# KUIS-AI-Tekalp-Research-Group/video-compression

Hardware: AMD Instinct MI355X
Metric: frames/sec + bpp/PSNR on UVG 1080p GOP-8, 1/2/4/8 MI355X (higher is better)
Workload: dtype f32; 1 GPU; LHBDC 1080p GOP-8 inference, single lambda: 7 B-frames per GOP via Model.forward, 4 independent GOP(s) per GPU per step, hierarchy levels batched across them; gop=8, resolution=1920x1080, precision=fp32, parallelism=gop-shard x1, launch=hip-graph per GOP pass

## Files before the change

video-compression_amd/csrc/conv_split.h:

```cpp
#pragma once
#include "conv_dma.h"

typedef short bf16x8 __attribute__((ext_vector_type(8)));

template <int K> struct SplitUnits {
    static constexpr int TPU = 4;
    static constexpr int Q = (K / 2) * (K / 2);
    static constexpr int V = (K + 3) / 4;
    static constexpr int H = (K - 1 + 3) / 4;
    static constexpr int U = Q + V + H;
    static constexpr int type(int u) { return u < Q ? 0 : (u < Q + V ? 1 : 2); }
    static constexpr int ky0(int u) { return u < Q ? 2 * (u / (K / 2)) : (u < Q + V ? 4 * (u - Q) : K - 1); }
    static constexpr int kx0(int u) { return u < Q ? 2 * (u % (K / 2)) : (u < Q + V ? K - 1 : 4 * (u - Q - V)); }
    static constexpr int nvalid(int u)
    {
        return u < Q ? 4 : (u < Q + V ? (K - 4 * (u - Q) < 4 ? K - 4 * (u - Q) : 4) : (K - 1 - 4 * (u - Q - V) < 4 ? K - 1 - 4 * (u - Q - V) : 4));
    }
    static constexpr int ky(int u, int q)
    {
        const int qq = q < nvalid(u) ? q : nvalid(u) - 1;
        return type(u) == 0 ? ky0(u) + (qq >> 1) : (type(u) == 1 ? ky0(u) + qq : ky0(u));
    }
    static constexpr int kx(int u, int q)
    {
        const int qq = q < nvalid(u) ? q : nvalid(u) - 1;
        return type(u) == 0 ? kx0(u) + (qq & 1) : (type(u) == 1 ? kx0(u) : kx0(u) + qq);
    }
    static constexpr bool valid(int u, int q) { return q < nvalid(u); }
    static constexpr int cls(int u) { return type(u) * 4 + nvalid(u) - 1; }
    static constexpr int NCLS = 12;
    static constexpr int dy(int c, int q)
    {
        const int t = c / 4, nv = c % 4 + 1, qq = q < nv ? q : nv - 1;
        return t == 0 ? (qq >> 1) : (t == 1 ? qq : 0);
    }
    static constexpr int dx(int c, int q)
    {
        const int t = c / 4, nv = c % 4 + 1, qq = q < nv ? q : nv - 1;
        return t == 0 ? (qq & 1) : (t == 1 ? 0 : qq);
    }
    static constexpr bool covers_all()
    {
        int seen[K * K] = {};
        for (int u = 0; u < U; ++u)
            for (int q = 0; q < 4; ++q)
                if (valid(u, q)) ++seen[ky(u, q) * K + kx(u, q)];
        for (int i = 0; i < K * K; ++i)
            if (seen[i] != 1) return false;
        return true;
    }
    static_assert(covers_all(), "every tap in exactly one unit");
};

template <int K> struct SplitPairs {
    static constexpr int TPU = 2;
    static constexpr int HP = (K - 1) / 2;
    static constexpr int Q = HP * K;
    static constexpr int V = (K + 1) / 2;
    static constexpr int U = Q + V;
    static constexpr int type(int u) { return u < Q ? 2 : 1; }
    static constexpr int ky0(int u) { return u < Q ? u / HP : 2 * (u - Q); }
    static constexpr int kx0(int u) { return u < Q ? 2 * (u % HP) : K - 1; }
    static constexpr int nvalid(int u) { return u < Q ? 2 : (K - 2 * (u - Q) < 2 ? 1 : 2); }
    static constexpr int ky(int u, int q) { return type(u) == 1 ? ky0(u) + (q < nvalid(u) ? q : nvalid(u) - 1) : ky0(u); }
    static constexpr int kx(int u, int q) { return type(u) == 2 ? kx0(u) + (q < nvalid(u) ? q : nvalid(u) - 1) : kx0(u); }
    static constexpr bool valid(int u, int q) { return q < nvalid(u); }
    static constexpr int cls(int u) { return type(u) * 4 + nvalid(u) - 1; }
    static constexpr int NCLS = 12;
    static constexpr int dy(int c, int q)
    {
        const int t = c / 4, nv = c % 4 + 1, qq = q < nv ? q : nv - 1;
        return t == 1 ? qq : 0;
    }
    static constexpr int dx(int c, int q)
    {
        const int t = c / 4, nv = c % 4 + 1, qq = q < nv ? q : nv - 1;
        return t == 2 ? qq : 0;
    }
    static constexpr bool covers_all()
    {
        int seen[K * K] = {};
        for (int u = 0; u < U; ++u)
            for (int q = 0; q < 2; ++q)
                if (valid(u, q)) ++seen[ky(u, q) * K + kx(u, q)];
        for (int i = 0; i < K * K; ++i)
            if (seen[i] != 1) return false;
        return true;
    }
    static_assert(covers_all(), "every tap in exactly one unit");
};

template <int K, int CPL> struct SplitUnitsOf { typedef SplitUnits<K> type; };
template <int K> struct SplitUnitsOf<K, 2> { typedef SplitPairs<K> type; };

template <int K_, int NTW_, int CPL_ = 1, int TH_ = 16, int RING_ = 4, int KO_ = 0> struct SplitCfg {
    typedef typename SplitUnitsOf<K_, CPL_>::type UN;
    static_assert(UN::TPU * CPL_ == 4, "four k-groups of 8 channels per MFMA");
    static constexpr int K = K_, NTW = NTW_, CPL = CPL_, RING = RING_, KO = KO_, U = UN::U, PAD = K_ / 2;
    static constexpr int TH = TH_, TW = 32, BN = 16 * NTW_;
    static constexpr int WAVES = 8, WM = TH_ * 2 / 8, WN = NTW_;
    static_assert(WM * 8 == TH_ * 2, "the tile's 2 TH M-tiles split evenly over 8 waves");
    static constexpr int ROWS_IN = TH + K_ - 1, COLS = TW + K_ - 1, PIX = ROWS_IN * COLS;
    static constexpr int PXB = 48;
    static constexpr int PLANE_SLOTS = CPL_ == 1 ? 3 * PIX : (3 * PIX + 15) / 16 * 16;
    static constexpr int PLANE_B = PLANE_SLOTS * 16;
    static constexpr int NA = (CPL_ * PLANE_SLOTS + 511) / 512;
    static constexpr int A_BYTES = NA * 8192;
    static constexpr int FRAGS = 3 * NTW_;
    static constexpr int ROUNDS = (FRAGS + 7) / 8, LASTW = FRAGS - 8 * (ROUNDS - 1);
    static constexpr bool EXACT = LASTW == 4;
    static constexpr int SLOTB = EXACT ? FRAGS * 1024 : ROUNDS * 8192;
    static constexpr int nb(int grp) { return ROUNDS - ((EXACT && grp == 1) ? 1 : 0); }
    static constexpr int B_OFF = 2 * A_BYTES, BIAS_OFF = B_OFF + RING_ * SLOTB;
    static constexpr int LDS_FIXED = BIAS_OFF;
    static constexpr int D = RING_ - 2;
    static constexpr int WIN = U - D - 1, PPP = (NA + WIN - 1) / WIN;
    static_assert(WIN >= 1, "no issue window for the chunk image");
    static constexpr int piece_phase(int k) { return 1 + k / PPP; }
    static constexpr int nA(int u)
    {
        int n = 0;
        for (int k = 0; k < NA; ++k) n += piece_phase(k) == u;
        return n;
    }
    static constexpr int nwait(int u, int grp)
    {
        int n = 0;
        for (int j = u + 2 - D; j <= u; ++j) n += nA(((j % U) + U) % U) + nb(grp);
        return n;
    }
    static_assert(D >= 1 && nwait(U - 1, 0) <= 63, "vmcnt is a 6-bit counter");
};

template <class C, int NG, int T0 = 0, int T1 = C::WM>
__device__ __forceinline__ void split_epilogue_records(const ConvArgs &p, f32x4 (&acc)[C::WM][C::WN], const DmaTile &cur, int wave, int px, int q,
                                                       unsigned char *sc)
{
    constexpr int WM = C::WM, WN = C::WN, UNITS = 96 * NG, NJ = (UNITS + 63) / 64, NGRP = (T1 - T0) * (WN / NG);
    static_assert(WN % NG == 0, "N-tiles are staged in whole groups");
    typedef unsigned u32x2 __attribute__((ext_vector_type(2)));
    const float neg = (p.act == VC_ACT_NONE) ? 1.0f : (p.act == VC_ACT_RELU ? 0.0f : p.slope);
    const int lane = px + 16 * q;
    int u_plane[NJ], u_w16[NJ];
#pragma unroll
    for (int j = 0; j < NJ; ++j) {
        const int u = 64 * j + lane;
        u_plane[j] = u / 48;
        u_w16[j] = u - 48 * u_plane[j];
    }
    unsigned char *const outb = reinterpret_cast<unsigned char *>(p.out) + (long long)cur.img * p.out_sn;
    const unsigned char *const resb = reinterpret_cast<const unsigned char *>(p.res) + (long long)cur.img * p.res_sn;
    auto unit_ok = [&](int g, int j, int &oy, int &oxb, int &plane0) {
        const int t = T0 + g / (WN / NG), n0 = (g % (WN / NG)) * NG, m = WM * wave + t;
        oy = cur.oy0 + (m >> 1);
        oxb = cur.ox0 + 16 * (m & 1);
        plane0 = (cur.nblk * C::BN + 16 * n0) >> 3;
        return (64 * j + lane < UNITS) && oy < p.Ho && (oxb + u_w16[j] / 3 < p.Wo);
    };
    vc_u32x4 rnext[NJ];
    auto fetch_res = [&](int g) {
#pragma unroll
        for (int j = 0; j < NJ; ++j) {
            int oy, oxb, plane0;
            const bool ok = unit_ok(g, j, oy, oxb, plane0);
            rnext[j] = vc_u32x4{0u, 0u, 0u, 0u};
            if (ok) rnext[j] = *reinterpret_cast<const vc_u32x4 *>(resb + ((((long long)(plane0 + u_plane[j])) * p.Ho + oy) * p.Wo + oxb) * 48 + u_w16[j] * 16);
        }
    };
    if (p.res_sp3) fetch_res(0);
#pragma unroll
    for (int g = 0; g < NGRP; ++g) {
        const int t = T0 + g / (WN / NG), n0 = (g % (WN / NG)) * NG;
        const int m = WM * wave + t;
        const int oy = cur.oy0 + (m >> 1), oxb = cur.ox0 + 16 * (m & 1), ox = oxb + px;
        const bool row_ok = oy < p.Ho, pix_ok = row_ok && ox < p.Wo;
        if (p.res_sp3) {
#pragma unroll
            for (int j = 0; j < NJ; ++j)
                if (64 * j + lane < UNITS) *reinterpret_cast<vc_u32x4 *>(sc + u_plane[j] * 768 + u_w16[j] * 16) = rnext[j];
            if (g + 1 < NGRP) fetch_res(g + 1);
            asm volatile("s_waitcnt lgkmcnt(0)" ::: "memory");
        }
#pragma unroll
        for (int nn = 0; nn < NG; ++nn) {
            const int n = n0 + nn;
            const int co = cur.nblk * C::BN + 16 * n + 4 * q;
            unsigned char *rec = sc + ((2 * nn + (q >> 1)) * 16 + px) * 48 + 8 * (q & 1);
            f32x4 v = acc[t][n];
            f32x4 r = {0.f, 0.f, 0.f, 0.f};
            if (p.res_sp3) {
                r = vc_load_split4(rec - 8 * (q & 1), q & 1);
            } else if (p.res) {
                if (pix_ok) r = *reinterpret_cast<const f32x4 *>(p.res + (long long)cur.img * p.res_sn + (long long)oy * p.res_sh + (long long)ox * p.res_sw + co);
            }
            if (p.res_first) v += r;
#pragma unroll
            for (int e = 0; e < 4; ++e) v[e] = v[e] >= 0.0f ? v[e] : v[e] * neg;
            if (p.chscale) v *= *reinterpret_cast<const f32x4 *>(p.chscale + co);
            if (p.res && !p.res_first) v += r;
            unsigned h[4], mm[4], l[4];
#pragma unroll
            for (int e = 0; e < 4; ++e) vc_split3(v[e], h[e], mm[e], l[e]);
            const u32x2 ph = {(h[0] >> 16) | h[1], (h[2] >> 16) | h[3]};
            const u32x2 pm = {(mm[0] >> 16) | mm[1], (mm[2] >> 16) | mm[3]};
            const u32x2 pl = {(l[0] >> 16) | (l[1] & 0xffff0000u), (l[2] >> 16) | (l[3] & 0xffff0000u)};
            if constexpr (C::KO & 256) {
                VC_DMA_KEEP(ph); VC_DMA_KEEP(pm); VC_DMA_KEEP(pl);
            } else {
                *reinterpret_cast<u32x2 *>(rec) = ph;
                *reinterpret_cast<u32x2 *>(rec + 16) = pm;
                *reinterpret_cast<u32x2 *>(rec + 32) = pl;
            }
        }
        if constexpr (C::KO & 256) continue;
        asm volatile("s_waitcnt lgkmcnt(0)" ::: "memory");
        const int plane0 = (cur.nblk * C::BN + 16 * n0) >> 3;
#pragma unroll
        for (int j = 0; j < NJ; ++j) {
            const bool ok = (64 * j + lane < UNITS) && row_ok && (oxb + u_w16[j] / 3 < p.Wo);
            if (ok) {
                const vc_u32x4 val = *reinterpret_cast<const vc_u32x4 *>(sc + u_plane[j] * 768 + u_w16[j] * 16);
                if constexpr (C::KO & 128) VC_DMA_KEEP(val);
                else *reinterpret_cast<vc_u32x4 *>(outb + ((((long long)(plane0 + u_plane[j])) * p.Ho + oy) * p.Wo + oxb) * 48 + u_w16[j] * 16) = val;
            }
        }
        asm volatile("s_waitcnt lgkmcnt(0)" ::: "memory");
    }
}

template <class C, int T0 = 0, int T1 = C::WM, int SC_NG = 0>
__device__ __forceinline__ void split_epilogue(const ConvArgs &p, f32x4 (&acc)[C::WM][C::WN], const DmaTile &cur, int wave, int px, int q,
                                               unsigned char *sc = nullptr)
{
    constexpr int WM = C::WM, WN = C::WN;
    if constexpr (SC_NG > 0 || (C::A_BYTES / 8 >= 3072 && WN % 2 == 0)) {
        if (sc && p.out_sp3 && p.out_mode == VC_OUT_PLAIN) {
            constexpr int NG = SC_NG > 0 ? SC_NG : ((C::A_BYTES / 8 >= WN * 1536) ? WN : 2);
            split_epilogue_records<C, NG, T0, T1>(p, acc, cur, wave, px, q, sc);
            return;
        }
    }
    const float neg = (p.act == VC_ACT_NONE) ? 1.0f : (p.act == VC_ACT_RELU ? 0.0f : p.slope);
#pragma unroll
    for (int t = T0; t < T1; ++t) {
        const int m = WM * wave + t;
        const int oy = cur.oy0 + (m >> 1), ox = cur.ox0 + 16 * (m & 1) + px;
        const bool pix_ok = oy < p.Ho && ox < p.Wo;
#pragma unroll
        for (int n = 0; n < WN; ++n) {
            const int co = cur.nblk * C::BN + 16 * n + 4 * q;
            const bool ok = pix_ok && co < p.Cout;
            f32x4 v = acc[t][n];
            f32x4 r = {0.f, 0.f, 0.f, 0.f};
            const bool ps = p.out_mode != VC_OUT_PLAIN;
            const int cps = p.Cout >> 2;
            const int pos = ps ? co / cps : 0;
            const int cch = ps ? co - pos * cps : co;
            const int yy = ps ? 2 * oy + (pos >> 1) : oy, xx = ps ? 2 * ox + (pos & 1) : ox;
            const int oh = ps ? 2 * p.Ho : p.Ho, ow = ps ? 2 * p.Wo : p.Wo;
            if (p.res_sp3) {
                if (ok) r = vc_load_split4(reinterpret_cast<const unsigned char *>(p.res) + (long long)cur.img * p.res_sn +
                                               ((((long long)(cch >> 3)) * oh + yy) * ow + xx) * 48, (cch >> 2) & 1);
            } else if (p.res) {
                const long long r_off = (long long)cur.img * p.res_sn + (long long)yy * p.res_sh + (long long)xx * p.res_sw + cch;
                if (ok) r = *reinterpret_cast<const f32x4 *>(p.res + r_off);
            }
            if (p.res_first) v += r;
#pragma unroll
            for (int e = 0; e < 4; ++e) v[e] = v[e] >= 0.0f ? v[e] : v[e] * neg;
            if (p.chscale) v *= *reinterpret_cast<const f32x4 *>(p.chscale + min(co, p.Cout - 4));
            if (p.res && !p.res_first) v += r;
            if (p.out_sp3) {
                unsigned char *o8 = reinterpret_cast<unsigned char *>(p.out) + (long long)cur.img * p.out_sn + ((((long long)(cch >> 3)) * oh + yy) * ow + xx) * 48;
                if (ok) vc_store_split4(o8, (cch >> 2) & 1, v);
            } else {
                const long long o_off = (long long)cur.img * p.out_sn + (long long)yy * p.out_sh + (long long)xx * p.out_sw + cch;
                if (ok) *reinterpret_cast<f32x4 *>(p.out + o_off) = v;
            }
        }
    }
}

template <class C> __global__ void __launch_bounds__(512, 2) conv_split_kernel(const ConvArgs p)
{
    typedef typename C::UN UN;
    constexpr int U = C::U, WM = C::WM, WN = C::WN, NA = C::NA, RING = C::RING, D = C::D, CPL = C::CPL;
    extern __shared__ __attribute__((aligned(16))) unsigned char lds8[];

    const int tid = threadIdx.x;
    const int lane = tid & 63;
    const int wave = __builtin_amdgcn_readfirstlane(tid >> 6);
    const int grp = wave >> 2;
    const int px = lane & 15, q = lane >> 4;

    const int per_img = p.tiles_x * p.tiles_y;
    const int total = per_img * p.N * p.nblks;
    const int xcd = blockIdx.x & 7, xl = blockIdx.x >> 3;
    const int tq = total >> 3, tr = total & 7;
    const int x_start = xcd * tq + min(xcd, tr), x_count = tq + (xcd < tr ? 1 : 0);
    auto tile_at = [&](int it) {
        DmaTile t;
        const int k = it * 32 + xl;
        t.valid = k < x_count;
        const int idx = x_start + (t.valid ? k : 0);
        t.nblk = idx % p.nblks;
        const int t1 = idx / p.nblks;
        t.img = t1 / per_img;
        int tx, ty;
        vc_tile_xy(t1 - t.img * per_img, p.tiles_x, p.tiles_y, p.tile_band, tx, ty);
        t.oy0 = ty * C::TH;
        t.ox0 = tx * C::TW;
        return t;
    };
    DmaTile cur = tile_at(0);
    if (!cur.valid) return;

    const int nchunk = p.Cin / (8 * CPL);
    const int upt = nchunk * U;
    const unsigned char *const in_b = reinterpret_cast<const unsigned char *>(p.in);
    const unsigned char *const wpk = reinterpret_cast<const unsigned char *>(p.wpk);
    const long long plane = (long long)p.H * p.W * C::PXB;
    const unsigned char *const zero_lane = g_vc_dma_zero + 16 * lane;

    int a_off[NA], a_rc[NA];
#pragma unroll
    for (int k = 0; k < NA; ++k) {
        const int s = k * 512 + tid;
        const int pl = s / C::PLANE_SLOTS, s2 = s - pl * C::PLANE_SLOTS;
        const int pix = s2 / 3, piece = s2 - 3 * pix;
        const int row = pix / C::COLS, col = pix - row * C::COLS;
        a_off[k] = pl * (int)plane + (row * p.W + col) * C::PXB + piece * 16;
        a_rc[k] = (pl < CPL && s2 < 3 * C::PIX) ? (row | (col << 8)) : 0x7f7f7f;
    }
    auto tile_base = [&](const DmaTile &t) {
        return in_b + (long long)t.img * p.in_sn + ((long long)(t.oy0 - C::PAD) * p.W + (t.ox0 - C::PAD)) * C::PXB;
    };
    auto issue_a = [&](const DmaTile &t, const unsigned char *tbase, int c, int k, int buf) {
        int rc = a_rc[k], off = a_off[k];
        asm volatile("" : "+v"(rc), "+v"(off));
        const unsigned iy = (unsigned)(t.oy0 - C::PAD + (rc & 0xff)), ix = (unsigned)(t.ox0 - C::PAD + (rc >> 8));
        const bool ok = t.valid && iy < (unsigned)p.H && ix < (unsigned)p.W;
        const unsigned char *sp = ok ? tbase + ((long long)c * CPL * plane + off) : zero_lane;
        if constexpr (!(C::KO & 16)) vc_glds16<true>(sp, (unsigned)(buf * C::A_BYTES + k * 8192 + wave * 1024));
    };
    const unsigned lane16 = 16 * lane;
    unsigned gbase = 0;
    auto issue_b = [&](int g, int nblk_cur, int nblk_next) {
        const int gg = g >= upt ? g - upt : g;
        const int nblk = g >= upt ? nblk_next : nblk_cur;
        const unsigned char *sbase = wpk + ((long long)nblk * upt + gg) * (C::FRAGS * 1024) + wave * 1024;
        const unsigned dst = C::B_OFF + ((gbase + (unsigned)g) % RING) * C::SLOTB + wave * 1024;
#pragma unroll
        for (int r = 0; r < C::ROUNDS; ++r)
            if constexpr (!(C::KO & 16)) {
                if (r + 1 < C::ROUNDS || !C::EXACT || grp == 0) vc_glds16_sbase(sbase + r * 8192, lane16, dst + r * 8192);
            }
    };

    float *const ldsf = reinterpret_cast<float *>(lds8);
    for (int i = tid; i < p.nblks * C::BN; i += 512) ldsf[C::BIAS_OFF / 4 + i] = p.bias[i];
    DmaTile nxt = tile_at(1);
    const unsigned char *cur_base = tile_base(cur), *nxt_base = tile_base(nxt);
#pragma unroll
    for (int k = 0; k < NA; ++k) issue_a(cur, cur_base, 0, k, 0);
#pragma unroll
    for (int g = 0; g < D; ++g) issue_b(g, cur.nblk, cur.nblk);
    vc_wait_vmcnt<0>();
    __syncthreads();

    constexpr bool TIMM = (WM % 2 == 0);
    const int qtap = q / CPL, qpl = q % CPL;
    int a_lane[UN::NCLS][TIMM ? 1 : WM];
#pragma unroll
    for (int c = 0; c < UN::NCLS; ++c) {
        int dy = 0, dx = 0;
#pragma unroll
        for (int qq = 0; qq < UN::TPU; ++qq)
            if (qtap == qq) {
                dy = UN::dy(c, qq);
                dx = UN::dx(c, qq);
            }
#pragma unroll
        for (int t = 0; t < (TIMM ? 1 : WM); ++t) {
            const int m = WM * wave + t;
            a_lane[c][t] = (((m >> 1) + dy) * C::COLS + 16 * (m & 1) + px + dx) * C::PXB + qpl * C::PLANE_B;
        }
    }
    const int b_lane = C::B_OFF + lane * 16;

    f32x4 acc[WM][WN];
    f32x4 af[3][WM], bf[3][WN];
    int gchunk = 0;
    for (int it = 0;; ++it) {
#pragma unroll
        for (int n = 0; n < WN; ++n) {
            const f32x4 b = *reinterpret_cast<const f32x4 *>(&ldsf[C::BIAS_OFF / 4 + cur.nblk * C::BN + 16 * n + 4 * q]);
#pragma unroll
            for (int t = 0; t < WM; ++t) acc[t][n] = b;
        }
        if (grp == 1) VC_DMA_BARRIER();
#pragma unroll 1
        for (int c = 0; c < nchunk; ++c) {
            const int abuf = ((gchunk + c) & 1) * C::A_BYTES, nbuf = ((gchunk + c + 1) & 1);
            const bool last_chunk = c + 1 == nchunk;
            const int g0 = c * U;
            static_for<0, U>([&](auto uc) {
                constexpr int u = decltype(uc)::value;
                constexpr int cl = UN::cls(u);
                const int bslot = b_lane + (int)((gbase + (unsigned)(g0 + u)) % RING) * C::SLOTB;
#pragma unroll
                for (int pc = 0; pc < 3; ++pc) {
#pragma unroll
                    for (int n = 0; n < WN; ++n) bf[pc][n] = *reinterpret_cast<const f32x4 *>(lds8 + bslot + (pc * WN + n) * 1024);
#pragma unroll
                    for (int t = 0; t < WM; ++t) {
                        const int ab = a_lane[cl][TIMM ? 0 : t] + abuf;
                        constexpr int unit_imm = (UN::ky0(u) * C::COLS + UN::kx0(u)) * C::PXB;
                        const int t_imm = TIMM ? ((t >> 1) * C::COLS + 16 * (t & 1)) * C::PXB : 0;
                        af[pc][t] = *reinterpret_cast<const f32x4 *>(lds8 + ab + unit_imm + t_imm + 16 * pc);
                    }
                }
                static_for<0, NA>([&](auto kc) {
                    constexpr int k = decltype(kc)::value;
                    if constexpr (C::piece_phase(k) == u) {
                        if (!last_chunk) issue_a(cur, cur_base, c + 1, k, nbuf);
                        else issue_a(nxt, nxt_base, 0, k, nbuf);
                    }
                });
                issue_b(g0 + u + D, cur.nblk, nxt.nblk);
                if constexpr (!(C::KO & 2)) {
                    if constexpr (C::nwait(u, 0) == C::nwait(u, 1)) vc_wait_vmcnt<C::nwait(u, 0)>();
                    else if (grp == 0) vc_wait_vmcnt<C::nwait(u, 0)>();
                    else vc_wait_vmcnt<C::nwait(u, 1)>();
                }
                VC_DMA_BARRIER();
                if constexpr (!(C::KO & 4)) {
                    __builtin_amdgcn_s_setprio(1);
#pragma unroll
                    for (int sum = 4; sum >= 0; --sum)
#pragma unroll
                        for (int pa = 2; pa >= 0; --pa) {
                            const int pb = sum - pa;
                            if (pb < 0 || pb > 2) continue;
#pragma unroll
                            for (int t = 0; t < WM; ++t)
#pragma unroll
                                for (int n = 0; n < WN; ++n)
                                    acc[t][n] = __builtin_amdgcn_mfma_f32_16x16x32_bf16(__builtin_bit_cast(bf16x8, bf[pb][n]),
                                                                                        __builtin_bit_cast(bf16x8, af[pa][t]), acc[t][n], 0, 0, 0);
                        }
                    __builtin_amdgcn_s_setprio(0);
                } else {
#pragma unroll
                    for (int pc = 0; pc < 3; ++pc) {
#pragma unroll
                        for (int t = 0; t < WM; ++t) VC_DMA_KEEP(af[pc][t]);
#pragma unroll
                        for (int n = 0; n < WN; ++n) VC_DMA_KEEP(bf[pc][n]);
                    }
                }
                VC_DMA_BARRIER();
            });
        }
        if (grp == 0) VC_DMA_BARRIER();
        gchunk += nchunk;
        gbase = (gbase + (unsigned)upt) % RING;

        if constexpr (!(C::KO & 1)) {
            split_epilogue<C>(p, acc, cur, wave, px, q);
        } else {
#pragma unroll
            for (int t = 0; t < WM; ++t)
#pragma unroll
                for (int n = 0; n < WN; ++n) VC_DMA_KEEP(acc[t][n]);
        }
        if (!nxt.valid) break;
        cur = nxt;
        cur_base = nxt_base;
        nxt = tile_at(it + 2);
        nxt_base = tile_base(nxt);
    }
    vc_wait_vmcnt<0>();
}

template <int K_, int NTW_, int TH_ = (K_ == 3 ? 12 : 16), int RING_ = 4, int KO_ = 0> struct SplitPeriodCfg {
    static constexpr int K = K_, NTW = NTW_, CPL = K_ == 3 ? 2 : 1, RING = RING_, KO = KO_, PAD = K_ / 2;
    static constexpr int KG = K_ * K_ * CPL, U = (2 * KG + 3) / 4;
    static constexpr int TH = TH_, TW = 32, BN = 16 * NTW_;
    static constexpr int WAVES = 8, WM = TH_ * 2 / 8, WN = NTW_;
    static_assert(WM * 8 == TH_ * 2, "the tile's 2 TH M-tiles split evenly over 8 waves");
    static constexpr int ROWS_IN = TH + K_ - 1, COLS = TW + K_ - 1, PIX = ROWS_IN * COLS, PXB = 48;
    static constexpr int PLANE_SLOTS = CPL == 1 ? 3 * PIX : (3 * PIX + 15) / 16 * 16, PLANE_B = PLANE_SLOTS * 16;
    static constexpr int NA = (CPL * PLANE_SLOTS + 511) / 512, A_BYTES = NA * 8192;
    static constexpr int FRAGS = 3 * NTW_, ROUNDS = (FRAGS + 7) / 8, LASTW = FRAGS - 8 * (ROUNDS - 1);
    static constexpr bool EXACT = LASTW == 4;
    static constexpr int SLOTB = EXACT ? FRAGS * 1024 : ROUNDS * 8192;
    static constexpr int nb(int grp) { return ROUNDS - ((EXACT && grp == 1) ? 1 : 0); }
    static constexpr int B_OFF = 2 * A_BYTES, BIAS_OFF = B_OFF + RING_ * SLOTB, LDS_FIXED = BIAS_OFF;
    static constexpr int D = RING_ - 2;
    static_assert(D == 2, "the issue windows below are laid out for weights requested two units ahead");
    static constexpr bool kg_valid(int u, int q) { return 4 * u + q < 2 * KG; }
    static constexpr int kg_chunk(int u, int q) { return kg_valid(u, q) ? (4 * u + q) / KG : 1; }
    static constexpr int kg_tap(int u, int q) { return kg_valid(u, q) ? ((4 * u + q) % KG) / CPL : 0; }
    static constexpr int kg_plane(int u, int q) { return kg_valid(u, q) ? ((4 * u + q) % KG) % CPL : 0; }
    static constexpr int XLAST = (KG - 1) / 4, YFIRST = KG / 4;
    static constexpr int YWIN = YFIRST - D, XWIN = U - D - XLAST - 1;
    static_assert(YWIN >= 1 && XWIN >= 1, "no issue window for a chunk image");
    static constexpr int PPP = (NA + (YWIN < XWIN ? YWIN : XWIN) - 1) / (YWIN < XWIN ? YWIN : XWIN);
    static constexpr int piece_phase(int which, int k) { return (which ? 1 : XLAST + 2) + k / PPP; }
    static_assert(piece_phase(1, NA - 1) <= YFIRST - D && piece_phase(0, NA - 1) <= U - D, "chunk image pieces outside their window");
    static constexpr int nA(int u)
    {
        int n = 0;
        for (int w = 0; w < 2; ++w)
            for (int k = 0; k < NA; ++k) n += piece_phase(w, k) == u;
        return n;
    }
    static constexpr int nwait(int u, int grp)
    {
        int n = 0;
        for (int j = u + 2 - D; j <= u; ++j) n += nA(((j % U) + U) % U) + nb(grp);
        return n;
    }
    static constexpr int max_wait()
    {
        int m = 0;
        for (int u = 0; u < U; ++u) m = nwait(u, 0) > m ? nwait(u, 0) : m;
        return m;
    }
    static_assert(max_wait() <= 63, "vmcnt is a 6-bit counter");
};

template <class C> __global__ void __launch_bounds__(512, 2) conv_split_period_kernel(const ConvArgs p)
{
    constexpr int U = C::U, WM = C::WM, WN = C::WN, NA = C::NA, RING = C::RING, D = C::D;
    extern __shared__ __attribute__((aligned(16))) unsigned char lds8[];
    const int tid = threadIdx.x;
    const int lane = tid & 63;
    const int wave = __builtin_amdgcn_readfirstlane(tid >> 6);
    const int grp = wave >> 2;
    const int px = lane & 15, q = lane >> 4;

    const int per_img = p.tiles_x * p.tiles_y;
    const int total = per_img * p.N * p.nblks;
    const int xcd = blockIdx.x & 7, xl = blockIdx.x >> 3;
    const int tq = total >> 3, tr = total & 7;
    const int x_start = xcd * tq + min(xcd, tr), x_count = tq + (xcd < tr ? 1 : 0);
    auto tile_at = [&](int it) {
        DmaTile t;
        const int k = it * 32 + xl;
        t.valid = k < x_count;
        const int idx = x_start + (t.valid ? k : 0);
        t.nblk = idx % p.nblks;
        const int t1 = idx / p.nblks;
        t.img = t1 / per_img;
        int tx, ty;
        vc_tile_xy(t1 - t.img * per_img, p.tiles_x, p.tiles_y, p.tile_band, tx, ty);
        t.oy0 = ty * C::TH;
        t.ox0 = tx * C::TW;
        return t;
    };
    DmaTile cur = tile_at(0);
    if (!cur.valid) return;

    const int nper = p.Cin / (16 * C::CPL);
    const int upt = nper * U;
    const unsigned char *const in_b = reinterpret_cast<const unsigned char *>(p.in);
    const unsigned char *const wpk = reinterpret_cast<const unsigned char *>(p.wpk);
    const long long plane = (long long)p.H * p.W * C::PXB;
    const unsigned char *const zero_lane = g_vc_dma_zero + 16 * lane;

    int a_off[NA], a_rc[NA];
#pragma unroll
    for (int k = 0; k < NA; ++k) {
        const int s = k * 512 + tid;
        const int pl = s / C::PLANE_SLOTS, s2 = s - pl * C::PLANE_SLOTS;
        const int pix = s2 / 3, piece = s2 - 3 * pix;
        const int row = pix / C::COLS, col = pix - row * C::COLS;
        a_off[k] = pl * (int)plane + (row * p.W + col) * C::PXB + piece * 16;
        a_rc[k] = (pl < C::CPL && s2 < 3 * C::PIX) ? (row | (col << 8)) : 0x7f7f7f;
    }
    auto tile_base = [&](const DmaTile &t) {
        return in_b + (long long)t.img * p.in_sn + ((long long)(t.oy0 - C::PAD) * p.W + (t.ox0 - C::PAD)) * C::PXB;
    };
    auto issue_a = [&](const DmaTile &t, const unsigned char *tbase, int c, int k, int buf) {
        int rc = a_rc[k], off = a_off[k];
        asm volatile("" : "+v"(rc), "+v"(off));
        const unsigned iy = (unsigned)(t.oy0 - C::PAD + (rc & 0xff)), ix = (unsigned)(t.ox0 - C::PAD + (rc >> 8));
        const bool ok = t.valid && iy < (unsigned)p.H && ix < (unsigned)p.W;
        const unsigned char *sp = ok ? tbase + ((long long)c * C::CPL * plane + off) : zero_lane;
        if constexpr (!(C::KO & 16)) vc_glds16<true>(sp, (unsigned)(buf * C::A_BYTES + k * 8192 + wave * 1024));
    };
    const unsigned lane16 = 16 * lane;
    unsigned gbase = 0;
    auto issue_b = [&](int g, int nblk_cur, int nblk_next) {
        const int gg = g >= upt ? g - upt : g;
        const int nblk = g >= upt ? nblk_next : nblk_cur;
        const unsigned char *sbase = wpk + ((long long)nblk * upt + gg) * (C::FRAGS * 1024) + wave * 1024;
        const unsigned dst = C::B_OFF + ((gbase + (unsigned)g) % RING) * C::SLOTB + wave * 1024;
#pragma unroll
        for (int r = 0; r < C::ROUNDS; ++r)
            if constexpr (!(C::KO & 16)) {
                if (r + 1 < C::ROUNDS || !C::EXACT || grp == 0) vc_glds16_sbase(sbase + r * 8192, lane16, dst + r * 8192);
            }
    };

    float *const ldsf = reinterpret_cast<float *>(lds8);
    for (int i = tid; i < p.nblks * C::BN; i += 512) ldsf[C::BIAS_OFF / 4 + i] = p.bias[i];
    DmaTile nxt = tile_at(1);
    const unsigned char *cur_base = tile_base(cur), *nxt_base = tile_base(nxt);
#pragma unroll
    for (int k = 0; k < NA; ++k) issue_a(cur, cur_base, 0, k, 0);
#pragma unroll
    for (int g = 0; g < D; ++g) issue_b(g, cur.nblk, cur.nblk);
    vc_wait_vmcnt<0>();
    __syncthreads();

    int a_t[WM], a_unit[U];
#pragma unroll
    for (int t = 0; t < WM; ++t) {
        const int m = WM * wave + t;
        a_t[t] = ((m >> 1) * C::COLS + 16 * (m & 1) + px) * C::PXB;
    }
#pragma unroll
    for (int u = 0; u < U; ++u) {
        int off = 0;
#pragma unroll
        for (int qq = 0; qq < 4; ++qq)
            if (q == qq)
                off = C::kg_chunk(u, qq) * C::A_BYTES + C::kg_plane(u, qq) * C::PLANE_B + ((C::kg_tap(u, qq) / C::K) * C::COLS + C::kg_tap(u, qq) % C::K) * C::PXB;
        a_unit[u] = off;
    }
    const int b_lane = C::B_OFF + lane * 16;

#ifdef VC_DMA_DIAG
    unsigned st_sum[8] = {0, 0, 0, 0, 0, 0, 0, 0};
#endif
    VC_DMA_STAMP(t_begin);
    f32x4 acc[WM][WN];
    f32x4 af[3][WM], bf[3][WN];
    for (int it = 0;; ++it) {
#pragma unroll
        for (int n = 0; n < WN; ++n) {
            const f32x4 b = *reinterpret_cast<const f32x4 *>(&ldsf[C::BIAS_OFF / 4 + cur.nblk * C::BN + 16 * n + 4 * q]);
#pragma unroll
            for (int t = 0; t < WM; ++t) acc[t][n] = b;
        }
        if (grp == 1) VC_DMA_BARRIER();
#pragma unroll 1
        for (int pr = 0; pr < nper; ++pr) {
            const bool last_per = pr + 1 == nper;
            const int g0 = pr * U;
            static_for<0, U>([&](auto uc) {
                constexpr int u = decltype(uc)::value;
                VC_DMA_STAMP(t0);
                const int bslot = b_lane + (int)((gbase + (unsigned)(g0 + u)) % RING) * C::SLOTB;
#pragma unroll
                for (int pc = 0; pc < 3; ++pc) {
#pragma unroll
                    for (int n = 0; n < WN; ++n) bf[pc][n] = *reinterpret_cast<const f32x4 *>(lds8 + bslot + (pc * WN + n) * 1024);
#pragma unroll
                    for (int t = 0; t < WM; ++t) af[pc][t] = *reinterpret_cast<const f32x4 *>(lds8 + (a_t[t] + a_unit[u]) + 16 * pc);
                }
                VC_DMA_STAMP(t1);
                static_for<0, NA>([&](auto kc) {
                    constexpr int k = decltype(kc)::value;
                    if constexpr (C::piece_phase(1, k) == u) issue_a(cur, cur_base, 2 * pr + 1, k, 1);
                    if constexpr (C::piece_phase(0, k) == u) {
                        if (!last_per) issue_a(cur, cur_base, 2 * pr + 2, k, 0);
                        else issue_a(nxt, nxt_base, 0, k, 0);
                    }
                });
                issue_b(g0 + u + D, cur.nblk, nxt.nblk);
                VC_DMA_STAMP(t2);
                if constexpr (!(C::KO & 2)) {
                    if constexpr (C::nwait(u, 0) == C::nwait(u, 1)) vc_wait_vmcnt<C::nwait(u, 0)>();
                    else if (grp == 0) vc_wait_vmcnt<C::nwait(u, 0)>();
                    else vc_wait_vmcnt<C::nwait(u, 1)>();
                }
                VC_DMA_STAMP(t3);
                VC_DMA_BARRIER();
                VC_DMA_STAMP(t4);
                if constexpr (!(C::KO & 4)) {
                    __builtin_amdgcn_s_setprio(1);
#pragma unroll
                    for (int sum = 4; sum >= 0; --sum)
#pragma unroll
                        for (int pa = 2; pa >= 0; --pa) {
                            const int pb = sum - pa;
                            if (pb < 0 || pb > 2) continue;
#pragma unroll
                            for (int t = 0; t < WM; ++t)
#pragma unroll
                                for (int n = 0; n < WN; ++n)
                                    acc[t][n] = __builtin_amdgcn_mfma_f32_16x16x32_bf16(__builtin_bit_cast(bf16x8, bf[pb][n]),
                                                                                        __builtin_bit_cast(bf16x8, af[pa][t]), acc[t][n], 0, 0, 0);
                        }
                    __builtin_amdgcn_s_setprio(0);
                } else {
#pragma unroll
                    for (int pc = 0; pc < 3; ++pc) {
#pragma unroll
                        for (int t = 0; t < WM; ++t) VC_DMA_KEEP(af[pc][t]);
#pragma unroll
                        for (int n = 0; n < WN; ++n) VC_DMA_KEEP(bf[pc][n]);
                    }
                }
                VC_DMA_STAMP(t5);
                VC_DMA_BARRIER();
                VC_DMA_STAMP(t6);
                VC_DMA_ACC(0, t2, t1);
                VC_DMA_ACC(1, t1, t0);
                VC_DMA_ACC(2, t3, t2);
                VC_DMA_ACC(3, t4, t3);
                VC_DMA_ACC(4, t5, t4);
                VC_DMA_ACC(5, t6, t5);
            });
        }
        if (grp == 0) VC_DMA_BARRIER();
        gbase = (gbase + (unsigned)upt) % RING;
        VC_DMA_STAMP(t_e0);
        if constexpr (!(C::KO & 1)) {
            split_epilogue<C>(p, acc, cur, wave, px, q, (C::KO & 32) ? nullptr : lds8 + C::A_BYTES + wave * (C::A_BYTES / 8));
        } else {
#pragma unroll
            for (int t = 0; t < WM; ++t)
#pragma unroll
                for (int n = 0; n < WN; ++n) VC_DMA_KEEP(acc[t][n]);
        }
        VC_DMA_STAMP(t_e1);
        VC_DMA_ACC(6, t_e1, t_e0);
        if (!nxt.valid) break;
        cur = nxt;
        cur_base = nxt_base;
        nxt = tile_at(it + 2);
        nxt_base = tile_base(nxt);
    }
    vc_wait_vmcnt<0>();
#ifdef VC_DMA_DIAG
    if constexpr (C::KO & 64) {
        VC_DMA_STAMP(t_end);
        st_sum[7] = t_end - t_begin;
        if (lane == 0)
            for (int i = 0; i < 8; ++i) atomicAdd(&g_vc_dma_stamps[i], (unsigned long long)st_sum[i]);
    }
#endif
}

template <class C> int launch_conv_split_period(hipStream_t st, const ConvArgs &a)
{
    const size_t lds_bytes = C::LDS_FIXED + (size_t)a.nblks * C::BN * sizeof(float);
    if (lds_bytes > 160 * 1024) return VC_EINVAL;
    auto kern = conv_split_period_kernel<C>;
    static vc_lds_raised raised;
    if (!vc_raise_lds_limit(reinterpret_cast<const void *>(kern), lds_bytes, raised)) return VC_ELAUNCH;
    hipLaunchKernelGGL(kern, dim3(256), dim3(512), lds_bytes, st, a);
    return hipGetLastError() == hipSuccess ? VC_OK : VC_ELAUNCH;
}

template <class C> int launch_conv_split(hipStream_t st, const ConvArgs &a)
{
    const size_t lds_bytes = C::LDS_FIXED + (size_t)a.nblks * C::BN * sizeof(float);
    if (lds_bytes > 160 * 1024) return VC_EINVAL;
    auto kern = conv_split_kernel<C>;
    static vc_lds_raised raised;
    if (!vc_raise_lds_limit(reinterpret_cast<const void *>(kern), lds_bytes, raised)) return VC_ELAUNCH;
    hipLaunchKernelGGL(kern, dim3(256), dim3(512), lds_bytes, st, a);
    return hipGetLastError() == hipSuccess ? VC_OK : VC_ELAUNCH;
}
```

video-compression_amd/csrc/conv_split.hip:

```cpp
#include <stdlib.h>
#include <string.h>
#include "conv_split.h"

static inline unsigned short bf16_trunc_bits(float x)
{
    unsigned u;
    memcpy(&u, &x, 4);
    return (unsigned short)(u >> 16);
}
static inline float bf16_bits_to_float(unsigned short h)
{
    const unsigned u = (unsigned)h << 16;
    float f;
    memcpy(&f, &u, 4);
    return f;
}
static inline void split3_host(float x, unsigned short pc[3])
{
    pc[0] = bf16_trunc_bits(x);
    const float r1 = x - bf16_bits_to_float(pc[0]);
    pc[1] = bf16_trunc_bits(r1);
    const float r2 = r1 - bf16_bits_to_float(pc[1]);
    pc[2] = bf16_trunc_bits(r2);
}

static int split_cpl(int k) { return k == 3 ? 2 : ((k == 5 || k == 7) ? 1 : 0); }
static int split_units(int k)
{
    return k == 7 ? SplitUnits<7>::U : (k == 5 ? SplitUnits<5>::U : (k == 3 ? SplitPairs<3>::U : 0));
}
static int split_block(int cout, int k)
{
    if (k == 3) return (cout % 64 == 0) ? 64 : ((cout % 32 == 0) ? 32 : 0);
    return (cout % 64 == 0) ? 64 : ((cout % 32 == 0) ? 32 : ((k == 7 && cout % 16 == 0) ? 16 : 0));
}

extern "C" size_t vc_conv_packed_weight_bytes_split(int cout, int cin, int k)
{
    const int u = split_units(k), bn = split_block(cout, k), cpl = split_cpl(k);
    if (!u || !bn || !cpl || (cin % (8 * cpl))) return 0;
    return (size_t)(cout / bn) * (cin / (8 * cpl)) * u * 3 * (bn / 16) * 1024 + 16384;
}

template <class UN, int K, int CPL> static void pack_split(const float *w, int cout, int cin, int bn, int ps, unsigned short *dst)
{
    const int ntw = bn / 16, nchunk = cin / (8 * CPL), cps = cout / 4;
    for (int nb = 0; nb < cout / bn; ++nb)
        for (int c = 0; c < nchunk; ++c)
            for (int u = 0; u < UN::U; ++u) {
                unsigned short *unit = dst + (((size_t)nb * nchunk + c) * UN::U + u) * (3 * ntw * 512);
                for (int n = 0; n < ntw; ++n)
                    for (int lane = 0; lane < 64; ++lane) {
                        const int cop = nb * bn + 16 * n + (lane & 15), q = lane >> 4;
                        const int co = ps ? (cop % cps) * 4 + cop / cps : cop;
                        const int tap = q / CPL, pl = q % CPL;
                        for (int j = 0; j < 8; ++j) {
                            unsigned short pc[3] = {0, 0, 0};
                            if (UN::valid(u, tap))
                                split3_host(w[(((size_t)co * cin + (c * CPL + pl) * 8 + j) * K + UN::ky(u, tap)) * K + UN::kx(u, tap)], pc);
                            for (int piece = 0; piece < 3; ++piece) unit[((piece * ntw + n) * 64 + lane) * 8 + j] = pc[piece];
                        }
                    }
            }
}

template <int K> static void pack_split_period(const float *w, int cout, int cin, int bn, int ps, unsigned short *dst)
{
    typedef SplitPeriodCfg<K, 4> C;
    constexpr int CPL = C::CPL, KG = C::KG, U = C::U;
    const int ntw = bn / 16, nper = cin / (16 * CPL), cps = cout / 4;
    for (int nb = 0; nb < cout / bn; ++nb)
        for (int pr = 0; pr < nper; ++pr)
            for (int u = 0; u < U; ++u) {
                unsigned short *unit = dst + (((size_t)nb * nper + pr) * U + u) * (3 * ntw * 512);
                for (int n = 0; n < ntw; ++n)
                    for (int lane = 0; lane < 64; ++lane) {
                        const int cop = nb * bn + 16 * n + (lane & 15), q = lane >> 4;
                        const int co = ps ? (cop % cps) * 4 + cop / cps : cop;
                        const int g = 4 * u + q;
                        if (g >= 2 * KG) continue;
                        const int chunk = g / KG, tap = (g % KG) / CPL, pl = (g % KG) % CPL;
                        for (int j = 0; j < 8; ++j) {
                            unsigned short pc[3];
                            split3_host(w[(((size_t)co * cin + (2 * pr + chunk) * 8 * CPL + 8 * pl + j) * K + tap / K) * K + tap % K], pc);
                            for (int piece = 0; piece < 3; ++piece) unit[((piece * ntw + n) * 64 + lane) * 8 + j] = pc[piece];
                        }
                    }
            }
}
static bool split_period(int k, int cin, int bn)
{
    if (bn == 16) return false;
    static const bool padded = [] {
        const char *e = getenv("VC_SPLIT_PADDED"), *e3 = getenv("VC_SPLIT3_PADDED");
        return (e && e[0] && e[0] != '0') || (e3 && e3[0] && e3[0] != '0');
    }();
    if (padded) return false;
    return (k == 3 && (cin % 32) == 0) || ((k == 5 || k == 7) && (cin % 16) == 0);
}

extern "C" int vc_conv_pack_weights_split(const float *w, const float *bias, int cout, int cin, int k, int pixelshuffle, void *wpk_out,
                                          float *bias_out)
{
    const size_t bytes = vc_conv_packed_weight_bytes_split(cout, cin, k);
    if (!w || !wpk_out || !bias_out || !bytes || (pixelshuffle && (cout % 16))) return VC_EINVAL;
    memset(wpk_out, 0, bytes);
    unsigned short *dst = static_cast<unsigned short *>(wpk_out);
    const int bn = split_block(cout, k);
    if (split_period(k, cin, bn)) {
        if (k == 7) pack_split_period<7>(w, cout, cin, bn, pixelshuffle, dst);
        else if (k == 5) pack_split_period<5>(w, cout, cin, bn, pixelshuffle, dst);
        else pack_split_period<3>(w, cout, cin, bn, pixelshuffle, dst);
    } else if (k == 7) pack_split<SplitUnits<7>, 7, 1>(w, cout, cin, bn, pixelshuffle, dst);
    else if (k == 5) pack_split<SplitUnits<5>, 5, 1>(w, cout, cin, bn, pixelshuffle, dst);
    else pack_split<SplitPairs<3>, 3, 2>(w, cout, cin, bn, pixelshuffle, dst);
    const int cps = cout / 4;
    for (int cop = 0; cop < cout; ++cop) {
        const int co = pixelshuffle ? (cop % cps) * 4 + cop / cps : cop;
        bias_out[cop] = bias ? bias[co] : 0.0f;
    }
    return VC_OK;
}

template <int PB> __global__ void __launch_bounds__(256) k_split3(vc_view a, unsigned char *__restrict__ out, long long out_img_bytes)
{
    __shared__ __attribute__((aligned(16))) unsigned char sm[VC_RECORDS_LDS(PB)];
    const int nb = (a.c >> 3) / PB;
    const int x_run = (int)blockIdx.x * (256 / PB);
    const int gi = threadIdx.x % PB, x = x_run + (int)threadIdx.x / PB, y = blockIdx.y;
    const int n = blockIdx.z / nb, g0 = (blockIdx.z - n * nb) * PB;
    vc_u32x4 ph = {0, 0, 0, 0}, pm = ph, pl = ph;
    if (x < a.w) {
        const float *src = a.p + view_off(a, n, y, x) + 8 * (g0 + gi);
        vc_split_record(*reinterpret_cast<const f32x4 *>(src), *reinterpret_cast<const f32x4 *>(src + 4), ph, pm, pl);
    }
    const long long plane_bytes = (long long)a.h * a.w * 48;
    vc_store_records_256<PB>(sm, threadIdx.x, x < a.w, ph, pm, pl, out + n * out_img_bytes + g0 * plane_bytes + ((long long)y * a.w + x_run) * 48,
                             plane_bytes, min(256 / PB, a.w - x_run));
}

extern "C" int vc_split3(vc_stream s, vc_view a, void *out_split, long long out_image_bytes)
{
    if (!a.p || !out_split || (a.c % 8) || (a.sw % 4) || (a.sh % 4) || (a.sn % 4) || ((uintptr_t)a.p % 16) || ((uintptr_t)out_split % 16) ||
        (out_image_bytes % 16))
        return VC_EINVAL;
    const long long total = (long long)a.n * (a.c / 8) * a.h * a.w;
    if (total <= 0) return VC_OK;
    const long long img = out_image_bytes ? out_image_bytes : (long long)(a.c / 8) * a.h * a.w * 48;
    unsigned char *o = static_cast<unsigned char *>(out_split);
    const int cg = a.c / 8;
    const int pb = cg % 8 == 0 ? 8 : (cg % 4 == 0 ? 4 : (cg % 2 == 0 ? 2 : 1));
    const long long gz = (long long)a.n * (cg / pb);
    if (a.h > 65535 || gz > 65535) return VC_EINVAL;
    const dim3 grid((unsigned)((a.w + 256 / pb - 1) / (256 / pb)), (unsigned)a.h, (unsigned)gz);
    if (pb == 8) hipLaunchKernelGGL(k_split3<8>, grid, dim3(256), 0, as_stream(s), a, o, img);
    else if (pb == 4) hipLaunchKernelGGL(k_split3<4>, grid, dim3(256), 0, as_stream(s), a, o, img);
    else if (pb == 2) hipLaunchKernelGGL(k_split3<2>, grid, dim3(256), 0, as_stream(s), a, o, img);
    else hipLaunchKernelGGL(k_split3<1>, grid, dim3(256), 0, as_stream(s), a, o, img);
    VC_LAUNCH_CHECK();
    return VC_OK;
}

int conv_dispatch_split(hipStream_t st, ConvArgs a, int k, int stride)
{
    const int cpl = split_cpl(k);
    if (stride != 1 || !cpl || !a.in_sp3 || a.in_f16 || a.out_f16 || a.res_f16 || a.tail_wpk || a.epi != VC_EPI_NONE || a.in_xform != VC_IN_NONE ||
        (a.Cin % (8 * cpl)) || a.act == VC_ACT_SIGMOID || a.act == VC_ACT_CLAMP01)
        return VC_EINVAL;
    const int bn = split_block(a.Cout, k);
    if (!bn) return VC_EINVAL;
    const int cpp = a.out_mode == VC_OUT_PLAIN ? a.Cout : a.Cout / 4;
    if (a.out_mode != VC_OUT_PLAIN && (a.Cout % 16)) return VC_EINVAL;
    if (a.out_sp3 ? (cpp % 8 != 0) : !a.vec_out) return VC_EINVAL;
    if ((long long)cpl * a.H * a.W * 48 + (long long)(k + 15) * a.W * 48 + 48ll * 48 >= (1ll << 31)) return VC_EINVAL;
    if (a.res_sp3 && (!a.res || (cpp % 8))) return VC_EINVAL;
    if (!a.in_sn) a.in_sn = (long long)(a.Cin / 8) * a.H * a.W * 48;
    const int osc = a.out_mode == VC_OUT_PLAIN ? 1 : 2;
    if (a.out_sp3 && !a.out_sn) a.out_sn = (long long)(cpp / 8) * osc * a.Ho * osc * a.Wo * 48;
    if (a.res_sp3 && !a.res_sn) a.res_sn = (long long)(cpp / 8) * osc * a.Ho * osc * a.Wo * 48;
    if ((a.in_sn % 16) || (a.out_sp3 && (a.out_sn % 16)) || (a.res_sp3 && (a.res_sn % 8))) return VC_EINVAL;
    const int th = k == 3 ? 12 : (bn == 16 ? 24 : 16);
    a.tiles_x = (a.Wo + 31) / 32;
    a.tiles_y = (a.Ho + th - 1) / th;
    a.nblks = a.Cout / bn;
    a.total_blocks = a.tiles_x * a.tiles_y * a.nblks * a.N;
#ifdef VC_SPLIT_DIAG
    {
        const char *e = getenv("VC_SPLIT_VARIANT");
        const int v = e ? atoi(e) : 0;
#ifdef VC_DMA_DIAG
        if (k == 3 && split_period(k, a.Cin, bn) && bn == 64) {
            if (v == 64 + 128) return launch_conv_split_period<SplitPeriodCfg<3, 4, 12, 4, 64 + 128>>(st, a);
            if (v == 64 + 256) return launch_conv_split_period<SplitPeriodCfg<3, 4, 12, 4, 64 + 256>>(st, a);
            if (v == 64 + 32) return launch_conv_split_period<SplitPeriodCfg<3, 4, 12, 4, 64 + 32>>(st, a);
        }
        if (v == 64 && split_period(k, a.Cin, bn) && bn == 64) {
            if (k == 3) return launch_conv_split_period<SplitPeriodCfg<3, 4, 12, 4, 64>>(st, a);
            if (k == 7) return launch_conv_split_period<SplitPeriodCfg<7, 4, 16, 4, 64>>(st, a);
        }
#endif
        if (k == 7 && bn == 64) {
            switch (v) {
            case 1: return launch_conv_split<SplitCfg<7, 4, 1, 16, 4, 1>>(st, a);
            case 4: return launch_conv_split<SplitCfg<7, 4, 1, 16, 4, 4>>(st, a);
            case 16: return launch_conv_split<SplitCfg<7, 4, 1, 16, 4, 16>>(st, a);
            case 17: return launch_conv_split<SplitCfg<7, 4, 1, 16, 4, 17>>(st, a);
            case 21: return launch_conv_split<SplitCfg<7, 4, 1, 16, 4, 21>>(st, a);
            }
        }
    }
#endif
    if (split_period(k, a.Cin, bn)) {
        if (k == 7) return bn == 64 ? launch_conv_split_period<SplitPeriodCfg<7, 4>>(st, a) : launch_conv_split_period<SplitPeriodCfg<7, 2>>(st, a);
        if (k == 5) return bn == 64 ? launch_conv_split_period<SplitPeriodCfg<5, 4>>(st, a) : launch_conv_split_period<SplitPeriodCfg<5, 2>>(st, a);
        return bn == 64 ? launch_conv_split_period<SplitPeriodCfg<3, 4>>(st, a) : launch_conv_split_period<SplitPeriodCfg<3, 2>>(st, a);
    }
    if (k == 7 && bn == 16) return launch_conv_split<SplitCfg<7, 1, 1, 24>>(st, a);
    if (k == 7) return bn == 64 ? launch_conv_split<SplitCfg<7, 4>>(st, a) : launch_conv_split<SplitCfg<7, 2>>(st, a);
    if (k == 5) return bn == 64 ? launch_conv_split<SplitCfg<5, 4>>(st, a) : launch_conv_split<SplitCfg<5, 2>>(st, a);
    if (k == 3) return bn == 64 ? launch_conv_split<SplitCfg<3, 4, 2, 12>>(st, a) : launch_conv_split<SplitCfg<3, 2, 2, 12>>(st, a);
    return VC_EINVAL;
}

#if defined(VC_SPLIT_DIAG) && defined(VC_DMA_DIAG)
extern "C" int vc_debug_dma_stamps(unsigned long long *out8)
{
    if (hipDeviceSynchronize() != hipSuccess) return VC_ELAUNCH;
    if (hipMemcpyFromSymbol(out8, HIP_SYMBOL(g_vc_dma_stamps), 8 * sizeof(unsigned long long)) != hipSuccess) return VC_ELAUNCH;
    unsigned long long zero[8] = {0};
    if (hipMemcpyToSymbol(HIP_SYMBOL(g_vc_dma_stamps), zero, sizeof(zero)) != hipSuccess) return VC_ELAUNCH;
    return VC_OK;
}
#endif
```

Before: 21.71 frames/s.

## Add wide 128-channel split-period conv tile for 3x3 layers with register bias

Adds a wide variant of the 3x3 split-period conv that covers 128 output channels with an 8-row tile instead of 64 channels with 12 rows. A heuristic picks it when its rounded work across 256-wide rounds is no larger. In the wide variant, bias lives in registers and is broadcast with ds_bpermute rather than staged in LDS. Weight fragments are gathered from two packed 64-channel units, so no repack is needed, and per-unit A offsets are computed inline to save registers. The aim is more weight reuse per loaded input tile and fewer input reloads, at the cost of higher register pressure and possibly lower occupancy. A residual-alignment guard is also added to the record epilogue.

After: 21.82 frames/s, median of 6. No clear change (+0.5%).

```diff
diff --git a/video-compression_amd/csrc/conv_split.h b/video-compression_amd/csrc/conv_split.h
--- a/video-compression_amd/csrc/conv_split.h
+++ b/video-compression_amd/csrc/conv_split.h
@@ -234,7 +234,8 @@
 {
     constexpr int WM = C::WM, WN = C::WN;
     if constexpr (SC_NG > 0 || (C::A_BYTES / 8 >= 3072 && WN % 2 == 0)) {
-        if (sc && p.out_sp3 && p.out_mode == VC_OUT_PLAIN) {
+        const bool res16 = !p.res_sp3 || (((unsigned long long)p.res_sn | (unsigned long long)reinterpret_cast<uintptr_t>(p.res)) & 15ull) == 0;
+        if (sc && p.out_sp3 && p.out_mode == VC_OUT_PLAIN && res16) {
             constexpr int NG = SC_NG > 0 ? SC_NG : ((C::A_BYTES / 8 >= WN * 1536) ? WN : 2);
             split_epilogue_records<C, NG, T0, T1>(p, acc, cur, wave, px, q, sc);
             return;
@@ -497,6 +498,16 @@
     static constexpr int SLOTB = EXACT ? FRAGS * 1024 : ROUNDS * 8192;
     static constexpr int nb(int grp) { return ROUNDS - ((EXACT && grp == 1) ? 1 : 0); }
     static constexpr int B_OFF = 2 * A_BYTES, BIAS_OFF = B_OFF + RING_ * SLOTB, LDS_FIXED = BIAS_OFF;
+    static constexpr bool BIAS_REG = NTW_ == 8;
+    static constexpr int SRC_NTW = NTW_ == 8 ? 4 : NTW_, SRC_FRAGS = 3 * SRC_NTW;
+    static_assert(NTW_ % SRC_NTW == 0 && (SRC_NTW == NTW_ || (!EXACT && LASTW == 8)), "a wide unit is whole rounds over whole packed units");
+    static constexpr int frag(int piece, int n) { return (n / SRC_NTW) * SRC_FRAGS + piece * SRC_NTW + n % SRC_NTW; }
+    static constexpr int unit_off(int u, int q) { return kg_chunk(u, q) * A_BYTES + kg_plane(u, q) * PLANE_B + ((kg_tap(u, q) / K_) * COLS + kg_tap(u, q) % K_) * PXB; }
+    static constexpr bool UNIT_OFF_REGS = NTW_ != 8;
+    static constexpr int LDS_MAX = 160 * 1024;
+    static_assert(LDS_FIXED <= LDS_MAX, "two chunk images and the weight ring must fit the CU's LDS");
+    static_assert(!BIAS_REG || BN == 128, "the register bias holds one block of 128 channels");
+    static_assert(A_BYTES / 8 >= 2 * 1536, "the record epilogue stages two N-tiles per wave in its eighth of buffer Y");
     static constexpr int D = RING_ - 2;
     static_assert(D == 2, "the issue windows below are laid out for weights requested two units ahead");
     static constexpr bool kg_valid(int u, int q) { return 4 * u + q < 2 * KG; }
@@ -601,12 +612,23 @@
 #pragma unroll
         for (int r = 0; r < C::ROUNDS; ++r)
             if constexpr (!(C::KO & 16)) {
-                if (r + 1 < C::ROUNDS || !C::EXACT || grp == 0) vc_glds16_sbase(sbase + r * 8192, lane16, dst + r * 8192);
+                if constexpr (C::SRC_NTW != C::NTW) {
+                    const int f = 8 * r + wave, half = f / C::SRC_FRAGS;
+                    const unsigned char *src = wpk + (((long long)(nblk * (C::NTW / C::SRC_NTW) + half) * upt + gg) * C::SRC_FRAGS + (f - half * C::SRC_FRAGS)) * 1024;
+                    vc_glds16_sbase(src, lane16, dst + r * 8192);
+                } else if (r + 1 < C::ROUNDS || !C::EXACT || grp == 0) vc_glds16_sbase(sbase + r * 8192, lane16, dst + r * 8192);
             }
     };
 
     float *const ldsf = reinterpret_cast<float *>(lds8);
-    for (int i = tid; i < p.nblks * C::BN; i += 512) ldsf[C::BIAS_OFF / 4 + i] = p.bias[i];
+    float bias_r[2] = {0.f, 0.f}, bias_n[2] = {0.f, 0.f};
+    auto load_bias = [&](float (&b)[2], int nblk) {
+        b[0] = p.bias[nblk * C::BN + lane];
+        b[1] = p.bias[nblk * C::BN + 64 + lane];
+    };
+    if constexpr (C::BIAS_REG) load_bias(bias_r, cur.nblk);
+    else
+        for (int i = tid; i < p.nblks * C::BN; i += 512) ldsf[C::BIAS_OFF / 4 + i] = p.bias[i];
     DmaTile nxt = tile_at(1);
     const unsigned char *cur_base = tile_base(cur), *nxt_base = tile_base(nxt);
 #pragma unroll
@@ -627,8 +649,7 @@
         int off = 0;
 #pragma unroll
         for (int qq = 0; qq < 4; ++qq)
-            if (q == qq)
-                off = C::kg_chunk(u, qq) * C::A_BYTES + C::kg_plane(u, qq) * C::PLANE_B + ((C::kg_tap(u, qq) / C::K) * C::COLS + C::kg_tap(u, qq) % C::K) * C::PXB;
+            if (q == qq) off = C::unit_off(u, qq);
         a_unit[u] = off;
     }
     const int b_lane = C::B_OFF + lane * 16;
@@ -642,7 +663,14 @@
     for (int it = 0;; ++it) {
 #pragma unroll
         for (int n = 0; n < WN; ++n) {
-            const f32x4 b = *reinterpret_cast<const f32x4 *>(&ldsf[C::BIAS_OFF / 4 + cur.nblk * C::BN + 16 * n + 4 * q]);
+            f32x4 b;
+            if constexpr (C::BIAS_REG) {
+#pragma unroll
+                for (int e = 0; e < 4; ++e)
+                    b[e] = __builtin_bit_cast(float, __builtin_amdgcn_ds_bpermute(4 * (16 * (n & 3) + 4 * q + e), __builtin_bit_cast(int, bias_r[n >> 2])));
+            } else {
+                b = *reinterpret_cast<const f32x4 *>(&ldsf[C::BIAS_OFF / 4 + cur.nblk * C::BN + 16 * n + 4 * q]);
+            }
 #pragma unroll
             for (int t = 0; t < WM; ++t) acc[t][n] = b;
         }
@@ -655,12 +683,20 @@
                 constexpr int u = decltype(uc)::value;
                 VC_DMA_STAMP(t0);
                 const int bslot = b_lane + (int)((gbase + (unsigned)(g0 + u)) % RING) * C::SLOTB;
+                int aoff;
+                if constexpr (C::UNIT_OFF_REGS) {
+                    aoff = a_unit[u];
+                } else {
+                    int qv = q;
+                    asm volatile("" : "+v"(qv));
+                    aoff = qv == 0 ? C::unit_off(u, 0) : (qv == 1 ? C::unit_off(u, 1) : (qv == 2 ? C::unit_off(u, 2) : C::unit_off(u, 3)));
+                }
 #pragma unroll
                 for (int pc = 0; pc < 3; ++pc) {
 #pragma unroll
-                    for (int n = 0; n < WN; ++n) bf[pc][n] = *reinterpret_cast<const f32x4 *>(lds8 + bslot + (pc * WN + n) * 1024);
-#pragma unroll
-                    for (int t = 0; t < WM; ++t) af[pc][t] = *reinterpret_cast<const f32x4 *>(lds8 + (a_t[t] + a_unit[u]) + 16 * pc);
+                    for (int n = 0; n < WN; ++n) bf[pc][n] = *reinterpret_cast<const f32x4 *>(lds8 + bslot + C::frag(pc, n) * 1024);
+#pragma unroll
+                    for (int t = 0; t < WM; ++t) af[pc][t] = *reinterpret_cast<const f32x4 *>(lds8 + (a_t[t] + aoff) + 16 * pc);
                 }
                 VC_DMA_STAMP(t1);
                 static_for<0, NA>([&](auto kc) {
@@ -720,6 +756,7 @@
         if (grp == 0) VC_DMA_BARRIER();
         gbase = (gbase + (unsigned)upt) % RING;
         VC_DMA_STAMP(t_e0);
+        if constexpr (C::BIAS_REG) load_bias(bias_n, nxt.nblk);
         if constexpr (!(C::KO & 1)) {
             split_epilogue<C>(p, acc, cur, wave, px, q, (C::KO & 32) ? nullptr : lds8 + C::A_BYTES + wave * (C::A_BYTES / 8));
         } else {
@@ -735,6 +772,10 @@
         cur_base = nxt_base;
         nxt = tile_at(it + 2);
         nxt_base = tile_base(nxt);
+        if constexpr (C::BIAS_REG) {
+            bias_r[0] = bias_n[0];
+            bias_r[1] = bias_n[1];
+        }
     }
     vc_wait_vmcnt<0>();
 #ifdef VC_DMA_DIAG
@@ -749,8 +790,8 @@
 
 template <class C> int launch_conv_split_period(hipStream_t st, const ConvArgs &a)
 {
-    const size_t lds_bytes = C::LDS_FIXED + (size_t)a.nblks * C::BN * sizeof(float);
-    if (lds_bytes > 160 * 1024) return VC_EINVAL;
+    const size_t lds_bytes = C::LDS_FIXED + (C::BIAS_REG ? 0 : (size_t)a.nblks * C::BN * sizeof(float));
+    if (lds_bytes > (size_t)C::LDS_MAX) return VC_EINVAL;
     auto kern = conv_split_period_kernel<C>;
     static vc_lds_raised raised;
     if (!vc_raise_lds_limit(reinterpret_cast<const void *>(kern), lds_bytes, raised)) return VC_ELAUNCH;
diff --git a/video-compression_amd/csrc/conv_split.hip b/video-compression_amd/csrc/conv_split.hip
--- a/video-compression_amd/csrc/conv_split.hip
+++ b/video-compression_amd/csrc/conv_split.hip
@@ -122,6 +122,17 @@
     return VC_OK;
 }
 
+static bool split_wide(const ConvArgs &a, int k, int bn)
+{
+    if (k != 3 || bn != 64 || (a.Cout % 128) || !split_period(k, a.Cin, bn)) return false;
+    const char *e = getenv("VC_SPLIT_WIDE");
+    if (e && e[0] == '0') return false;
+    if (e && e[0] == '1') return true;
+    const long long tx = (a.Wo + 31) / 32;
+    auto rounds = [&](int th, int blk) { return ((long long)a.N * ((a.Ho + th - 1) / th) * tx * (a.Cout / blk) + 255) / 256; };
+    return rounds(8, 128) * 8 * 128 <= rounds(12, 64) * 12 * 64;
+}
+
 template <int PB> __global__ void __launch_bounds__(256) k_split3(vc_view a, unsigned char *__restrict__ out, long long out_img_bytes)
 {
     __shared__ __attribute__((aligned(16))) unsigned char sm[VC_RECORDS_LDS(PB)];
@@ -167,8 +178,10 @@
     if (stride != 1 || !cpl || !a.in_sp3 || a.in_f16 || a.out_f16 || a.res_f16 || a.tail_wpk || a.epi != VC_EPI_NONE || a.in_xform != VC_IN_NONE ||
         (a.Cin % (8 * cpl)) || a.act == VC_ACT_SIGMOID || a.act == VC_ACT_CLAMP01)
         return VC_EINVAL;
-    const int bn = split_block(a.Cout, k);
+    int bn = split_block(a.Cout, k);
     if (!bn) return VC_EINVAL;
+    const bool wide = split_wide(a, k, bn);
+    if (wide) bn = 128;
     const int cpp = a.out_mode == VC_OUT_PLAIN ? a.Cout : a.Cout / 4;
     if (a.out_mode != VC_OUT_PLAIN && (a.Cout % 16)) return VC_EINVAL;
     if (a.out_sp3 ? (cpp % 8 != 0) : !a.vec_out) return VC_EINVAL;
@@ -179,11 +192,12 @@
     if (a.out_sp3 && !a.out_sn) a.out_sn = (long long)(cpp / 8) * osc * a.Ho * osc * a.Wo * 48;
     if (a.res_sp3 && !a.res_sn) a.res_sn = (long long)(cpp / 8) * osc * a.Ho * osc * a.Wo * 48;
     if ((a.in_sn % 16) || (a.out_sp3 && (a.out_sn % 16)) || (a.res_sp3 && (a.res_sn % 8))) return VC_EINVAL;
-    const int th = k == 3 ? 12 : (bn == 16 ? 24 : 16);
+    const int th = wide ? 8 : (k == 3 ? 12 : (bn == 16 ? 24 : 16));
     a.tiles_x = (a.Wo + 31) / 32;
     a.tiles_y = (a.Ho + th - 1) / th;
     a.nblks = a.Cout / bn;
     a.total_blocks = a.tiles_x * a.tiles_y * a.nblks * a.N;
+    if (wide) return launch_conv_split_period<SplitPeriodCfg<3, 8, 8>>(st, a);
 #ifdef VC_SPLIT_DIAG
     {
         const char *e = getenv("VC_SPLIT_VARIANT");
```
